# rknightion/iq-to-audio

Hardware: AMD Instinct MI355X
Metric: complex IQ MS/s end-to-end (ingest->48 kHz audio) (higher is better)
Workload: dtype i8; 1 GPU; BASELINE config 2: synthetic 60 s @ 10 MS/s int16 I/Q, 1 NFM channel, +25 kHz, bw 12.5 kHz, D=104, 6401 taps, chunk 4194304; frames_per_gpu=600000000, parallelism=1 independent capture(s), one per GPU; RCCL gather of 48 kHz audio only, audio_samples_48k=2879996, mix_sign=1, settle_steps=55

## Files before the change

### iq-to-audio_amd/csrc/demod_fused.hip

```cpp
#include "common.h"

namespace iqa {

constexpr int SC_THREADS = 256;
constexpr int SC_ITEMS = 8;
constexpr int SC_TILE = SC_THREADS * SC_ITEMS;

struct Aff {
    double A, B;
};
__device__ __forceinline__ Aff then(const Aff &l, const Aff &r) { return Aff{r.A * l.A, fma(r.A, l.B, r.B)}; }

__device__ __forceinline__ Aff wave_inclusive(Aff v, int lane)
{
#pragma unroll
    for (int o = 1; o < kWave; o <<= 1) {
        const double la = __shfl_up(v.A, o, kWave);
        const double lb = __shfl_up(v.B, o, kWave);
        if (lane >= o) v = then(Aff{la, lb}, v);
    }
    return v;
}

__device__ __forceinline__ long long lower_bound_ll(const long long *arr, long long n, long long v)
{
    long long lo = 0, hi = n;
    while (lo < hi) {
        const long long mid = (lo + hi) >> 1;
        if (arr[mid] < v) lo = mid + 1; else hi = mid;
    }
    return lo;
}

enum FOp { F_DEEMPH = 0, F_DC = 1, F_AGC = 2 };
enum FSrc { S_F32 = 0, S_QUAD = 1, S_ENV = 2, S_REAL = 3 };
enum FSink { K_PLAIN = 0, K_CLIP = 1 };

struct FusedArgs {
    const float2 *z;
    const float *x;
    float *y;
    long long n;
    double p0, p1;
    const float2 *prev;
    const double *st;
    const long long *segs;
    long long n_segs;
    unsigned int *peak_bits;
    double *sumsq;
    Aff *agg;
    double *carry;
    double *fin;
    int nblocks;
    int z_aligned, y_aligned;
    int fresh;
};

template <int SRC>
__device__ __forceinline__ float src_value(float2 zc, float2 zp)
{
    if constexpr (SRC == S_QUAD) {
        const float re = zc.x * zp.x + zc.y * zp.y;
        const float im = zc.y * zp.x - zc.x * zp.y;
        return atan2f(im, re);
    } else if constexpr (SRC == S_ENV) {
        return np_abs_c64(zc.x, zc.y);
    } else {
        return zc.x;
    }
}


__global__ void k_quadrature(const float2 *z, long long n, const float2 *prev, float *out)
{
    const long long i = static_cast<long long>(blockIdx.x) * blockDim.x + threadIdx.x;
    if (i >= n) return;
    out[i] = src_value<S_QUAD>(z[i], (i == 0) ? prev[0] : z[i - 1]);
}

__global__ void k_store_last(const float2 *z, long long n, float2 *prev)
{
    if (threadIdx.x == 0 && blockIdx.x == 0) prev[0] = z[n - 1];
}

__global__ void k_envelope(const float2 *z, long long n, float *out)
{
    const long long i = static_cast<long long>(blockIdx.x) * blockDim.x + threadIdx.x;
    if (i < n) out[i] = src_value<S_ENV>(z[i], z[i]);
}

__global__ void k_real(const float2 *z, long long n, float *out)
{
    const long long i = static_cast<long long>(blockIdx.x) * blockDim.x + threadIdx.x;
    if (i < n) out[i] = src_value<S_REAL>(z[i], z[i]);
}


template <int OP, int SRC>
__device__ __forceinline__ void load_u(const FusedArgs &a, long long base, float (&u)[SC_ITEMS], float &u_before)
{
    u_before = 0.f;
    if constexpr (SRC == S_F32) {
#pragma unroll
        for (int i = 0; i < SC_ITEMS; ++i) u[i] = (base + i < a.n) ? a.x[base + i] : 0.f;
        if constexpr (OP == F_DC) {
            if (base == 0) u_before = a.fresh ? 0.f : static_cast<float>(a.st[0]);
            else if (base - 1 < a.n) u_before = a.x[base - 1];
        }
    } else {
        float2 zz[SC_ITEMS + 2];
        static_assert(SC_ITEMS == 8, "the vector path below moves 8 float2 = 4 x 16 bytes per thread");
        const int lane = threadIdx.x & 63;
        const long long wave_base = base - static_cast<long long>(lane) * SC_ITEMS;
        if (a.z_aligned && wave_base + 64 * SC_ITEMS <= a.n) {
            const float4 *p = reinterpret_cast<const float4 *>(a.z + base);
            const float4 q0 = p[0], q1 = p[1], q2 = p[2], q3 = p[3];
            zz[2] = make_float2(q0.x, q0.y);
            zz[3] = make_float2(q0.z, q0.w);
            zz[4] = make_float2(q1.x, q1.y);
            zz[5] = make_float2(q1.z, q1.w);
            zz[6] = make_float2(q2.x, q2.y);
            zz[7] = make_float2(q2.z, q2.w);
            zz[8] = make_float2(q3.x, q3.y);
            zz[9] = make_float2(q3.z, q3.w);
            float2 e0 = make_float2(0.f, 0.f), e1 = make_float2(0.f, 0.f);
            if (lane == 0 && base >= 2) {
                e0 = a.z[base - 2];
                e1 = a.z[base - 1];
            }
            zz[0] = make_float2(__shfl_up(q3.x, 1, kWave), __shfl_up(q3.y, 1, kWave));
            zz[1] = make_float2(__shfl_up(q3.z, 1, kWave), __shfl_up(q3.w, 1, kWave));
            if (lane == 0) {
                zz[0] = e0;
                zz[1] = e1;
            }
        } else {
#pragma unroll
            for (int i = 0; i < SC_ITEMS + 2; ++i) {
                const long long k = base - 2 + i;
                zz[i] = (k >= 0 && k < a.n) ? a.z[k] : make_float2(0.f, 0.f);
            }
        }
        if constexpr (SRC == S_QUAD) {
            if (base == 0) zz[1] = a.fresh ? make_float2(1.f, 0.f) : a.prev[0];
        }
#pragma unroll
        for (int i = 0; i < SC_ITEMS; ++i) u[i] = (base + i < a.n) ? src_value<SRC>(zz[i + 2], zz[i + 1]) : 0.f;
        if constexpr (OP == F_DC) {
            if (base == 0) u_before = a.fresh ? 0.f : static_cast<float>(a.st[0]);
            else u_before = src_value<SRC>(zz[1], zz[0]);
        }
    }
}

template <int OP>
__device__ __forceinline__ Aff fmap(const FusedArgs &a, long long idx, float x, float x_prev, bool maybe_reset)
{
    if constexpr (OP == F_DEEMPH) {
        return Aff{a.p0, a.p1 * static_cast<double>(x)};
    } else if constexpr (OP == F_DC) {
        return Aff{a.p0, static_cast<double>(x - x_prev)};
    } else {
        const float mag = fabsf(x);
        Aff m{1.0, 0.0};
        if (mag > 1e-6f) {
            const float desired = static_cast<float>(a.p0) / mag;
            m = Aff{1.0 - a.p1, a.p1 * static_cast<double>(desired)};
        }
        if (maybe_reset) {
            bool rst = (idx == 0);
            if (!rst && a.segs != nullptr && a.n_segs > 0) {
                const long long lo = lower_bound_ll(a.segs, a.n_segs, idx);
                rst = lo < a.n_segs && a.segs[lo] == idx;
            }
            if (rst) m = Aff{0.0, m.A + m.B};
        }
        return m;
    }
}

__device__ __forceinline__ bool block_has_restart(const FusedArgs &a, long long lo_i, long long hi_i)
{
    if (lo_i == 0) return true;
    if (a.segs == nullptr || a.n_segs <= 0) return false;
    const long long lo = lower_bound_ll(a.segs, a.n_segs, lo_i);
    return lo < a.n_segs && a.segs[lo] < hi_i;
}


template <int THREADS>
__device__ __forceinline__ void sink_count_segments(const FusedArgs &a, long long seg_first, long long first, long long last,
                                                    long long *s_seg)
{
    const int tid = threadIdx.x, lane = tid & 63;
    int c0 = (tid < a.n_segs) && seg_first <= first, c1 = (tid < a.n_segs) && seg_first <= last;
    for (long long kk = tid + THREADS; kk < a.n_segs; kk += THREADS) {
        const long long st = a.segs[kk];
        c0 += st <= first;
        c1 += st <= last;
    }
    c0 = static_cast<int>(wave_sum(static_cast<float>(c0)));
    c1 = static_cast<int>(wave_sum(static_cast<float>(c1)));
    if (lane == 0 && (c0 | c1)) {
        atomicAdd(reinterpret_cast<unsigned long long *>(&s_seg[0]), static_cast<unsigned long long>(c0));
        atomicAdd(reinterpret_cast<unsigned long long *>(&s_seg[1]), static_cast<unsigned long long>(c1));
    }
}

struct SinkPlan {
    bool stats, uniform, simple, general;
    long long seg0, seg1, bnd;
    int sub;
};
__device__ __forceinline__ SinkPlan sink_plan(const FusedArgs &a, bool stats, const long long *s_seg)
{
    SinkPlan p;
    p.stats = stats;
    p.seg0 = stats ? s_seg[0] : -1;
    p.seg1 = stats ? s_seg[1] : -1;
    p.uniform = stats && (p.seg0 == p.seg1);
    p.simple = stats && (p.seg1 == p.seg0 + 1);
    p.general = stats && !p.uniform && !p.simple;
    p.bnd = a.n;
    if (p.simple) p.bnd = a.segs[p.seg1];
    p.sub = blockIdx.x & (IQA_SUMSQ_SLOTS - 1);
    return p;
}

struct SinkAcc {
    float pk = 0.f;
    double run = 0.0, run_hi = 0.0;
    long long seg = 0;
};

template <int SINK>
__device__ __forceinline__ float sink_item(const FusedArgs &a, const SinkPlan &p, SinkAcc &k, float v, long long idx)
{
    if constexpr (SINK != K_CLIP) return v;
    k.pk = fmaxf(k.pk, fabsf(v));
    if (p.stats) {
        const double vv = static_cast<double>(v) * static_cast<double>(v);
        double run = k.run, run_hi = k.run_hi;
        long long seg = k.seg;
        if (p.general) {
            while (seg + 1 < a.n_segs && a.segs[seg + 1] <= idx) {
                if (run != 0.0) atomicAdd(&a.sumsq[seg * IQA_SUMSQ_SLOTS + p.sub], run);
                run = 0.0;
                ++seg;
            }
            run += vv;
        } else {
            const bool low = idx < p.bnd;
            run += low ? vv : 0.0;
            run_hi += low ? 0.0 : vv;
        }
        k.run = run;
        k.run_hi = run_hi;
        k.seg = seg;
    }
    return fminf(fmaxf(v, -0.99f), 0.99f);
}

__device__ __forceinline__ void sink_flush_general(const FusedArgs &a, const SinkPlan &p, SinkAcc &k)
{
    if (p.general && k.run != 0.0) atomicAdd(&a.sumsq[k.seg * IQA_SUMSQ_SLOTS + p.sub], k.run);
    if (p.general) k.run = 0.0;
}

template <int WAVES>
__device__ __forceinline__ void sink_finish(const FusedArgs &a, const SinkPlan &p, SinkAcc &k, float *s_pk, double *s_sq)
{
    const int tid = threadIdx.x, lane = tid & 63, wave = tid >> 6;
    sink_flush_general(a, p, k);
    const float pk = wave_max(k.pk);
    const double wlo = (p.stats && !p.general) ? wave_sum(k.run) : 0.0;
    const double whi = p.simple ? wave_sum(k.run_hi) : 0.0;
    if (lane == 0) {
        s_pk[wave] = pk;
        s_sq[wave] = wlo;
        s_sq[WAVES + wave] = whi;
    }
    __syncthreads();
    if (tid == 0) {
        float m = s_pk[0];
        double lo = s_sq[0], hi = s_sq[WAVES];
#pragma unroll
        for (int w = 1; w < WAVES; ++w) {
            m = fmaxf(m, s_pk[w]);
            lo += s_sq[w];
            hi += s_sq[WAVES + w];
        }
        if (a.peak_bits != nullptr) {
            const unsigned int mb = __float_as_uint(m);
            if (mb > __hip_atomic_load(a.peak_bits, __ATOMIC_RELAXED, __HIP_MEMORY_SCOPE_AGENT)) atomicMax(a.peak_bits, mb);
        }
        if (p.stats && !p.general) atomicAdd(&a.sumsq[p.seg0 * IQA_SUMSQ_SLOTS + p.sub], lo);
        if (p.simple) atomicAdd(&a.sumsq[p.seg1 * IQA_SUMSQ_SLOTS + p.sub], hi);
    }
}

__device__ __forceinline__ void store_items(const FusedArgs &a, long long base, long long lo, long long hi, const float (&vout)[SC_ITEMS])
{
    if (a.y_aligned && base >= lo && base + SC_ITEMS <= hi) {
        float4 *yp = reinterpret_cast<float4 *>(a.y + base);
        yp[0] = make_float4(vout[0], vout[1], vout[2], vout[3]);
        yp[1] = make_float4(vout[4], vout[5], vout[6], vout[7]);
    } else {
#pragma unroll
        for (int i = 0; i < SC_ITEMS; ++i)
            if (base + i >= lo && base + i < hi) a.y[base + i] = vout[i];
    }
}

template <int OP, int SRC>
__global__ __launch_bounds__(SC_THREADS) void k_fused_reduce(FusedArgs a)
{
    __shared__ Aff s_w[SC_THREADS / kWave];
    const int tid = threadIdx.x, lane = tid & 63, wave = tid >> 6;
    const long long blk0 = static_cast<long long>(blockIdx.x) * SC_TILE;
    const long long base = blk0 + static_cast<long long>(tid) * SC_ITEMS;
    const bool mr = (OP == F_AGC) && block_has_restart(a, blk0, blk0 + SC_TILE);
    float u[SC_ITEMS], ub;
    load_u<OP, SRC>(a, base, u, ub);
    Aff t{1.0, 0.0};
#pragma unroll
    for (int i = 0; i < SC_ITEMS; ++i)
        if (base + i < a.n) t = then(t, fmap<OP>(a, base + i, u[i], i ? u[i - 1] : ub, mr));
    const Aff inc = wave_inclusive(t, lane);
    if (lane == kWave - 1) s_w[wave] = inc;
    __syncthreads();
    if (tid == 0) {
        Aff tot = s_w[0];
#pragma unroll
        for (int w = 1; w < SC_THREADS / kWave; ++w) tot = then(tot, s_w[w]);
        a.agg[blockIdx.x] = tot;
    }
}

constexpr int FC_THREADS = 1024;
template <int OP>
__global__ __launch_bounds__(FC_THREADS) void k_fused_carry(FusedArgs a)
{
    __shared__ Aff s_w[FC_THREADS / kWave];
    const int tid = threadIdx.x, lane = tid & 63, wave = tid >> 6;
    double s0;
    if constexpr (OP == F_DEEMPH) s0 = a.fresh ? 0.0 : a.st[0];
    else if constexpr (OP == F_DC) s0 = a.fresh ? 0.0 : a.st[1];
    else s0 = 1.0;
    const int per = (a.nblocks + FC_THREADS - 1) / FC_THREADS;
    const int b0 = tid * per;
    Aff t{1.0, 0.0};
    for (int i = 0; i < per; ++i)
        if (b0 + i < a.nblocks) t = then(t, a.agg[b0 + i]);
    const Aff inc = wave_inclusive(t, lane);
    if (lane == kWave - 1) s_w[wave] = inc;
    __syncthreads();
    Aff pre{1.0, 0.0};
    for (int w = 0; w < wave; ++w) pre = then(pre, s_w[w]);
    Aff exl{__shfl_up(inc.A, 1, kWave), __shfl_up(inc.B, 1, kWave)};
    if (lane == 0) exl = Aff{1.0, 0.0};
    const Aff ex = then(pre, exl);
    double s = fma(ex.A, s0, ex.B);
    for (int i = 0; i < per; ++i) {
        const int b = b0 + i;
        if (b < a.nblocks) {
            a.carry[b] = s;
            const Aff v = a.agg[b];
            s = fma(v.A, s, v.B);
        }
    }
    if (tid == FC_THREADS - 1) a.fin[0] = s;
    if (a.fresh) {
        if (tid == 0 && a.peak_bits != nullptr) a.peak_bits[0] = 0u;
        if (a.sumsq != nullptr)
            for (long long i = tid; i < a.n_segs * IQA_SUMSQ_SLOTS; i += FC_THREADS) a.sumsq[i] = 0.0;
    }
    if (tid == 0) {
        if (a.prev != nullptr) reinterpret_cast<float2 *>(a.fin + 1)[0] = a.fresh ? make_float2(1.f, 0.f) : a.prev[0];
        if (a.st != nullptr) a.fin[2] = a.fresh ? 0.0 : a.st[0];
    }
}

template <int OP, int SRC, int SINK>
__global__ __launch_bounds__(SC_THREADS) void k_fused_apply(FusedArgs a, float2 *prev_out, double *st_out)
{
    __shared__ Aff s_w[SC_THREADS / kWave];
    __shared__ float s_pk[SC_THREADS / kWave];
    __shared__ double s_sq[2 * (SC_THREADS / kWave)];
    __shared__ long long s_seg[2];
    const int tid = threadIdx.x, lane = tid & 63, wave = tid >> 6;
    const long long blk0 = static_cast<long long>(blockIdx.x) * SC_TILE;
    const long long base = blk0 + static_cast<long long>(tid) * SC_ITEMS;
    const bool mr = (OP == F_AGC) && block_has_restart(a, blk0, blk0 + SC_TILE);
    const bool stats = (SINK == K_CLIP) && a.sumsq != nullptr && a.n_segs > 0;
    const double carry_in = a.carry[blockIdx.x];
    long long seg_first = 0;
    if (stats && tid < a.n_segs) seg_first = a.segs[tid];
    if (stats && tid < 2) s_seg[tid] = -1;
    float u[SC_ITEMS], ub;
    load_u<OP, SRC>(a, base, u, ub);
    constexpr bool KEEP = (OP == F_AGC);
    Aff m[KEEP ? SC_ITEMS : 1];
    Aff t{1.0, 0.0};
#pragma unroll
    for (int i = 0; i < SC_ITEMS; ++i) {
        const Aff mi = (base + i < a.n) ? fmap<OP>(a, base + i, u[i], i ? u[i - 1] : ub, mr) : Aff{1.0, 0.0};
        if constexpr (KEEP) m[i] = mi;
        t = then(t, mi);
    }
    if (stats) {
        __syncthreads();
        const long long first = blk0, last = min(blk0 + SC_TILE, a.n) - 1;
        int c0 = (tid < a.n_segs) && seg_first <= first, c1 = (tid < a.n_segs) && seg_first <= last;
        for (long long kk = tid + SC_THREADS; kk < a.n_segs; kk += SC_THREADS) {
            const long long st = a.segs[kk];
            c0 += st <= first;
            c1 += st <= last;
        }
        c0 = static_cast<int>(wave_sum(static_cast<float>(c0)));
        c1 = static_cast<int>(wave_sum(static_cast<float>(c1)));
        if (lane == 0 && (c0 | c1)) {
            atomicAdd(reinterpret_cast<unsigned long long *>(&s_seg[0]), static_cast<unsigned long long>(c0));
            atomicAdd(reinterpret_cast<unsigned long long *>(&s_seg[1]), static_cast<unsigned long long>(c1));
        }
    }
    const Aff inc = wave_inclusive(t, lane);
    if (lane == kWave - 1) s_w[wave] = inc;
    __syncthreads();
    const double ea = __shfl_up(inc.A, 1, kWave), eb = __shfl_up(inc.B, 1, kWave);
    Aff ex = (lane == 0) ? Aff{1.0, 0.0} : Aff{ea, eb};
    Aff wpre{1.0, 0.0};
    for (int w = 0; w < wave; ++w) wpre = then(wpre, s_w[w]);
    ex = then(wpre, ex);
    double s = fma(ex.A, carry_in, ex.B);

    const long long seg0 = stats ? s_seg[0] : -1, seg1 = stats ? s_seg[1] : -1;
    const bool uniform = stats && (seg0 == seg1);
    const bool simple = stats && (seg1 == seg0 + 1);
    const bool general = stats && !uniform && !simple;
    long long bnd = a.n;
    if (simple) bnd = a.segs[seg1];
    long long seg = seg0;
    if (general && base < a.n) seg = lower_bound_ll(a.segs, a.n_segs, base + 1) - 1;
    float pk = 0.f;
    double run = 0.0, run_hi = 0.0;
    float vout[SC_ITEMS];
#pragma unroll
    for (int i = 0; i < SC_ITEMS; ++i) {
        const long long idx = base + i;
        Aff mi;
        if constexpr (KEEP) mi = m[i];
        else mi = (idx < a.n) ? fmap<OP>(a, idx, u[i], i ? u[i - 1] : ub, mr) : Aff{1.0, 0.0};
        s = fma(mi.A, s, mi.B);
        vout[i] = 0.f;
        if (idx < a.n) {
            const float v = (OP == F_AGC) ? u[i] * static_cast<float>(s) : static_cast<float>(s);
            if constexpr (SINK == K_CLIP) {
                pk = fmaxf(pk, fabsf(v));
                vout[i] = fminf(fmaxf(v, -0.99f), 0.99f);
                if (stats) {
                    const double vv = static_cast<double>(v) * static_cast<double>(v);
                    if (general) {
                        while (seg + 1 < a.n_segs && a.segs[seg + 1] <= idx) {
                            if (run != 0.0) atomicAdd(&a.sumsq[seg * IQA_SUMSQ_SLOTS + (blockIdx.x & (IQA_SUMSQ_SLOTS - 1))], run);
                            run = 0.0;
                            ++seg;
                        }
                        run += vv;
                    } else {
                        run += idx < bnd ? vv : 0.0;
                        run_hi += idx < bnd ? 0.0 : vv;
                    }
                }
            } else {
                vout[i] = v;
            }
        }
    }
    if constexpr (SINK == K_CLIP) {
        if (general && run != 0.0) atomicAdd(&a.sumsq[seg * IQA_SUMSQ_SLOTS + (blockIdx.x & (IQA_SUMSQ_SLOTS - 1))], run);
        pk = wave_max(pk);
        const double wlo = (stats && !general) ? wave_sum(run) : 0.0;
        const double whi = simple ? wave_sum(run_hi) : 0.0;
        if (lane == 0) {
            s_pk[wave] = pk;
            s_sq[wave] = wlo;
            s_sq[4 + wave] = whi;
        }
        __syncthreads();
        if (tid == 0) {
            if (a.peak_bits != nullptr) {
                const unsigned int m = __float_as_uint(fmaxf(fmaxf(s_pk[0], s_pk[1]), fmaxf(s_pk[2], s_pk[3])));
                if (m > __hip_atomic_load(a.peak_bits, __ATOMIC_RELAXED, __HIP_MEMORY_SCOPE_AGENT)) atomicMax(a.peak_bits, m);
            }
            const int sub = blockIdx.x & (IQA_SUMSQ_SLOTS - 1);
            if (stats && !general) atomicAdd(&a.sumsq[seg0 * IQA_SUMSQ_SLOTS + sub], s_sq[0] + s_sq[1] + s_sq[2] + s_sq[3]);
            if (simple) atomicAdd(&a.sumsq[seg1 * IQA_SUMSQ_SLOTS + sub], s_sq[4] + s_sq[5] + s_sq[6] + s_sq[7]);
        }
    }
    if (OP != F_AGC && blockIdx.x == a.nblocks - 1 && tid == 0) {
        if constexpr (SRC == S_QUAD) prev_out[0] = a.z[a.n - 1];
        if constexpr (OP == F_DEEMPH) {
            st_out[0] = a.fin[0];
        } else if constexpr (OP == F_DC) {
            float last;
            if constexpr (SRC == S_F32) last = a.x[a.n - 1];
            else last = src_value<SRC>(a.z[a.n - 1], make_float2(0.f, 0.f));
            st_out[0] = static_cast<double>(last);
            st_out[1] = a.fin[0];
        }
    }
    if (a.y_aligned && base + SC_ITEMS <= a.n) {
        float4 *yp = reinterpret_cast<float4 *>(a.y + base);
        yp[0] = make_float4(vout[0], vout[1], vout[2], vout[3]);
        yp[1] = make_float4(vout[4], vout[5], vout[6], vout[7]);
    } else {
#pragma unroll
        for (int i = 0; i < SC_ITEMS; ++i)
            if (base + i < a.n) a.y[base + i] = vout[i];
    }
}

constexpr int FW_THREADS = 256;
constexpr int FW_ROUNDS = 4;
constexpr int FW_WAVES = FW_THREADS / kWave;
constexpr long long FW_ROUND = static_cast<long long>(FW_THREADS) * SC_ITEMS;
constexpr long long FW_SPAN = FW_ROUND * FW_ROUNDS;

static int scan_window(double alpha, long long *window)
{
    if (!(alpha > 0.0 && alpha < 1.0)) return 1;
    const double need = 64.0 * log(2.0) / -log(alpha);
    if (!(need < static_cast<double>(FW_SPAN))) return 1;
    long long w = 512 * static_cast<long long>(ceil(need / 512.0));
    if (w < 512) w = 512;
    while (w > 512 && pow(alpha, static_cast<double>(w - 512)) <= 0x1p-64) w -= 512;
    while (pow(alpha, static_cast<double>(w)) > 0x1p-64) w += 512;
    if (2 * w > FW_SPAN) return 1;
    *window = w;
    return 0;
}

template <int SRC>
__device__ __forceinline__ double windowed_round(const FusedArgs &a, long long base, long long end, bool skip0, Aff *s_w,
                                                 double &s_run, float (&u)[SC_ITEMS])
{
    const int lane = threadIdx.x & 63, wave = threadIdx.x >> 6;
    float ub;
    load_u<F_DEEMPH, SRC>(a, base, u, ub);
    if (skip0 && base == 0) u[0] = 0.f;
    Aff t{1.0, 0.0};
#pragma unroll
    for (int i = 0; i < SC_ITEMS; ++i)
        if (base + i < end) t = then(t, fmap<F_DEEMPH>(a, base + i, u[i], 0.f, false));
    const Aff inc = wave_inclusive(t, lane);
    if (lane == kWave - 1) s_w[wave] = inc;
    __syncthreads();
    const double ea = __shfl_up(inc.A, 1, kWave), eb = __shfl_up(inc.B, 1, kWave);
    Aff ex = (lane == 0) ? Aff{1.0, 0.0} : Aff{ea, eb};
    Aff acc{1.0, 0.0}, wpre{1.0, 0.0};
#pragma unroll
    for (int w = 0; w < FW_WAVES; ++w) {
        if (w == wave) wpre = acc;
        acc = then(acc, s_w[w]);
    }
    ex = then(wpre, ex);
    const double s = fma(ex.A, s_run, ex.B);
    s_run = fma(acc.A, s_run, acc.B);
    return s;
}

__global__ __launch_bounds__(FC_THREADS) void k_fused_clear(float *state, unsigned int *peak_bits, double *sumsq, long long n_sums)
{
    if (state != nullptr && threadIdx.x < 8) state[threadIdx.x] = threadIdx.x ? 0.f : 1.f;
    if (threadIdx.x == 0 && peak_bits != nullptr) peak_bits[0] = 0u;
    if (sumsq != nullptr)
        for (long long i = threadIdx.x; i < n_sums; i += FC_THREADS) sumsq[i] = 0.0;
}

template <int SRC, int SINK>
__global__ __launch_bounds__(FW_THREADS) void k_fused_windowed(FusedArgs a, long long window, float2 *prev_out, double *st_out)
{
    __shared__ Aff s_w[2][FW_WAVES];
    __shared__ float s_pk[FW_WAVES];
    __shared__ double s_sq[2 * FW_WAVES];
    __shared__ long long s_seg[2];
    const int tid = threadIdx.x;
    const long long own = FW_SPAN - window;
    const long long own0 = static_cast<long long>(blockIdx.x) * own, own1 = min(own0 + own, a.n);
    const long long start = blockIdx.x ? own0 - window : 0;
    const bool skip0 = blockIdx.x != 0;
    const bool stats = (SINK == K_CLIP) && a.sumsq != nullptr && a.n_segs > 0;
    double s_run = (blockIdx.x == 0 && !a.fresh) ? a.st[0] : 0.0;
    long long seg_first = 0;
    if (stats && tid < a.n_segs) seg_first = a.segs[tid];
    if (stats && tid < 2) s_seg[tid] = -1;
    if (stats) {
        __syncthreads();
        sink_count_segments<FW_THREADS>(a, seg_first, own0, own1 - 1, s_seg);
    }
    SinkPlan plan{};
    SinkAcc acc;
    for (int r = 0; r < FW_ROUNDS; ++r) {
        const long long rbase = start + r * FW_ROUND;
        if (rbase >= own1) break;
        const long long base = rbase + static_cast<long long>(tid) * SC_ITEMS;
        float u[SC_ITEMS];
        double s = windowed_round<SRC>(a, base, own1, skip0, s_w[r & 1], s_run, u);
        if (r == 0) plan = sink_plan(a, stats, s_seg);
        if (base + SC_ITEMS <= own0 || base >= own1) continue;
        acc.seg = plan.seg0;
        if (plan.general) acc.seg = lower_bound_ll(a.segs, a.n_segs, max(base, own0) + 1) - 1;
        float vout[SC_ITEMS];
#pragma unroll
        for (int i = 0; i < SC_ITEMS; ++i) {
            const long long idx = base + i;
            if (idx < own1) {
                const Aff mi = fmap<F_DEEMPH>(a, idx, u[i], 0.f, false);
                s = fma(mi.A, s, mi.B);
            }
            vout[i] = 0.f;
            if (idx >= own0 && idx < own1) vout[i] = sink_item<SINK>(a, plan, acc, static_cast<float>(s), idx);
        }
        sink_flush_general(a, plan, acc);
        store_items(a, base, own0, own1, vout);
    }
    if constexpr (SINK == K_CLIP) sink_finish<FW_WAVES>(a, plan, acc, s_pk, s_sq);
    if (blockIdx.x != 0) return;
    if (a.nblocks > 1) {
        const long long t0 = (a.n - window) & ~7LL;
        s_run = 0.0;
        __syncthreads();
        for (int r = 0; t0 + r * FW_ROUND < a.n; ++r) {
            float u[SC_ITEMS];
            windowed_round<SRC>(a, t0 + r * FW_ROUND + static_cast<long long>(tid) * SC_ITEMS, a.n, false, s_w[r & 1], s_run, u);
        }
    }
    if (tid == 0) {
        if constexpr (SRC == S_QUAD) prev_out[0] = a.z[a.n - 1];
        st_out[0] = s_run;
    }
}

template <int OP, int SRC, int SINK>
static int launch_fused(FusedArgs a, float2 *prev_out, double *st_out, void *work, hipStream_t s)
{
    if constexpr (OP == F_DEEMPH) {
        long long window;
        if (scan_window(a.p0, &window) == 0) {
            const long long own = FW_SPAN - window;
            a.nblocks = static_cast<int>((a.n + own - 1) / own);
            if (a.fresh && (a.peak_bits != nullptr || a.sumsq != nullptr))
                hipLaunchKernelGGL(k_fused_clear, dim3(1), dim3(FC_THREADS), 0, s, static_cast<float *>(nullptr), a.peak_bits, a.sumsq,
                                   a.n_segs * IQA_SUMSQ_SLOTS);
            hipLaunchKernelGGL((k_fused_windowed<SRC, SINK>), dim3(a.nblocks), dim3(FW_THREADS), 0, s, a, window, prev_out, st_out);
            return check_launch("windowed demodulator");
        }
    }
    a.nblocks = static_cast<int>((a.n + SC_TILE - 1) / SC_TILE);
    char *w = static_cast<char *>(work);
    a.agg = reinterpret_cast<Aff *>(w);
    a.carry = reinterpret_cast<double *>(w + sizeof(Aff) * a.nblocks);
    a.fin = a.carry + a.nblocks;
    hipLaunchKernelGGL((k_fused_reduce<OP, SRC>), dim3(a.nblocks), dim3(SC_THREADS), 0, s, a);
    hipLaunchKernelGGL((k_fused_carry<OP>), dim3(1), dim3(FC_THREADS), 0, s, a);
    FusedArgs b = a;
    b.prev = reinterpret_cast<const float2 *>(a.fin + 1);
    b.st = a.fin + 2;
    b.fresh = 0;
    hipLaunchKernelGGL((k_fused_apply<OP, SRC, SINK>), dim3(a.nblocks), dim3(SC_THREADS), 0, s, b, prev_out, st_out);
    return check_launch("fused demodulator");
}

}

using namespace iqa;

static int demodulate(const iqa_demod_params *p, const void *z_dev, int64_t n, void *state_dev, const void *seg_starts_dev,
                      int64_t n_segs, void *peak_dev, void *sumsq_dev, void *audio_out_dev, void *scratch_dev, void *work_dev,
                      void *stream, int fresh)
{
    if (p == nullptr) return fail_inval("params is NULL");
    if (n < 0 || n_segs < 0) return fail_inval("negative length");
    if (p->mode < IQA_DEMOD_NFM || p->mode > IQA_DEMOD_LSB) return fail_inval("Unsupported demod mode");
    if (n == 0) return IQA_OK;
    if (!z_dev || !state_dev || !audio_out_dev || !work_dev) return fail_inval("NULL device pointer");
    if (n_segs > 0 && !seg_starts_dev) return fail_inval("seg_starts is NULL");
    hipStream_t s = as_stream(stream);
    char *st = static_cast<char *>(state_dev);
    FusedArgs a{};
    a.fresh = fresh;
    a.z = static_cast<const float2 *>(z_dev);
    a.n = n;
    a.segs = static_cast<const long long *>(seg_starts_dev);
    a.n_segs = n_segs;
    a.peak_bits = static_cast<unsigned int *>(peak_dev);
    a.sumsq = static_cast<double *>(sumsq_dev);
    a.y = static_cast<float *>(audio_out_dev);
    a.z_aligned = (reinterpret_cast<uintptr_t>(z_dev) & 15) == 0;
    a.y_aligned = (reinterpret_cast<uintptr_t>(audio_out_dev) & 15) == 0;
    a.prev = reinterpret_cast<const float2 *>(st);
    if (p->mode == IQA_DEMOD_NFM) {
        a.p0 = p->deemph_alpha;
        a.p1 = 1.0 - p->deemph_alpha;
        a.st = reinterpret_cast<const double *>(st + 8);
        return launch_fused<F_DEEMPH, S_QUAD, K_CLIP>(a, reinterpret_cast<float2 *>(st), reinterpret_cast<double *>(st + 8),
                                                      work_dev, s);
    }
    if (!(p->dc_radius > 0.0 && p->dc_radius < 1.0)) return fail_inval("radius must be between 0 and 1");
    a.p0 = static_cast<double>(static_cast<float>(p->dc_radius));
    a.st = reinterpret_cast<const double *>(st + 16);
    double *dc_out = reinterpret_cast<double *>(st + 16);
    if (p->mode == IQA_DEMOD_AM) return launch_fused<F_DC, S_ENV, K_CLIP>(a, nullptr, dc_out, work_dev, s);
    if (!p->agc_enabled) return launch_fused<F_DC, S_REAL, K_CLIP>(a, nullptr, dc_out, work_dev, s);
    if (!scratch_dev) return fail_inval("SSB with AGC needs a float scratch buffer of n elements");
    FusedArgs d = a;
    d.y = static_cast<float *>(scratch_dev);
    d.y_aligned = (reinterpret_cast<uintptr_t>(scratch_dev) & 15) == 0;
    d.peak_bits = nullptr;
    d.sumsq = nullptr;
    int rc = launch_fused<F_DC, S_REAL, K_PLAIN>(d, nullptr, dc_out, work_dev, s);
    if (rc != IQA_OK) return rc;
    FusedArgs g = a;
    g.z = nullptr;
    g.x = static_cast<const float *>(scratch_dev);
    g.p0 = static_cast<double>(static_cast<float>(p->agc_target));
    g.p1 = static_cast<double>(static_cast<float>(p->agc_decay));
    g.st = nullptr;
    return launch_fused<F_AGC, S_F32, K_CLIP>(g, nullptr, nullptr, work_dev, s);
}

extern "C" int iqa_demodulate(const iqa_demod_params *p, const void *z_dev, int64_t n, void *state_dev,
                              const void *seg_starts_dev, int64_t n_segs, void *peak_dev, void *sumsq_dev,
                              void *audio_out_dev, void *scratch_dev, void *work_dev, void *stream)
{
    return demodulate(p, z_dev, n, state_dev, seg_starts_dev, n_segs, peak_dev, sumsq_dev, audio_out_dev, scratch_dev, work_dev, stream, 0);
}

extern "C" int iqa_demodulate_from_reset(const iqa_demod_params *p, const void *z_dev, int64_t n, void *state_dev,
                                         const void *seg_starts_dev, int64_t n_segs, void *peak_dev, void *sumsq_dev,
                                         void *audio_out_dev, void *scratch_dev, void *work_dev, void *stream)
{
    if (n == 0) return fail_inval("iqa_demodulate_from_reset needs samples (an empty block resets nothing)");
    return demodulate(p, z_dev, n, state_dev, seg_starts_dev, n_segs, peak_dev, sumsq_dev, audio_out_dev, scratch_dev, work_dev, stream, 1);
}

extern "C" int iqa_demod_reset(void *state_dev, void *peak_dev, void *sumsq_dev, int64_t n_sums, void *stream)
{
    if (n_sums < 0) return fail_inval("negative length");
    if (!state_dev) return fail_inval("NULL device pointer");
    if (n_sums > 0 && !sumsq_dev) return fail_inval("sumsq is NULL");
    hipLaunchKernelGGL(k_fused_clear, dim3(1), dim3(FC_THREADS), 0, as_stream(stream), static_cast<float *>(state_dev),
                       static_cast<unsigned int *>(peak_dev), static_cast<double *>(sumsq_dev), (long long)n_sums);
    return check_launch("k_fused_clear");
}

extern "C" int iqa_scan_window(double alpha, int64_t *window, int64_t *span)
{
    long long w = 0;
    if (scan_window(alpha, &w) != 0) return 1;
    if (window != nullptr) *window = w;
    if (span != nullptr) *span = FW_SPAN;
    return 0;
}

extern "C" int64_t iqa_scan_workspace_bytes(int64_t n)
{
    const int64_t nb = (n + SC_TILE - 1) / SC_TILE;
    return nb * (sizeof(Aff) + sizeof(double)) + 64;
}


static FusedArgs stage_args(const void *x_dev, int64_t n, void *y_dev)
{
    FusedArgs a{};
    a.x = static_cast<const float *>(x_dev);
    a.y = static_cast<float *>(y_dev);
    a.n = n;
    a.y_aligned = (reinterpret_cast<uintptr_t>(y_dev) & 15) == 0;
    return a;
}

extern "C" int iqa_deemphasis(const void *x_dev, int64_t n, double alpha, void *state_dev, void *y_dev,
                              void *work_dev, void *stream)
{
    if (n < 0) return fail_inval("negative length");
    if (n == 0) return IQA_OK;
    if (!x_dev || !state_dev || !y_dev || !work_dev) return fail_inval("NULL device pointer");
    FusedArgs a = stage_args(x_dev, n, y_dev);
    a.p0 = alpha;
    a.p1 = 1.0 - alpha;
    a.st = static_cast<const double *>(state_dev);
    return launch_fused<F_DEEMPH, S_F32, K_PLAIN>(a, nullptr, static_cast<double *>(state_dev), work_dev, as_stream(stream));
}

extern "C" int iqa_dc_block(const void *x_dev, int64_t n, double radius, void *state_dev, void *y_dev,
                            void *work_dev, void *stream)
{
    if (n < 0) return fail_inval("negative length");
    if (!(radius > 0.0 && radius < 1.0)) return fail_inval("radius must be between 0 and 1");
    if (n == 0) return IQA_OK;
    if (!x_dev || !state_dev || !y_dev || !work_dev) return fail_inval("NULL device pointer");
    FusedArgs a = stage_args(x_dev, n, y_dev);
    a.p0 = static_cast<double>(static_cast<float>(radius));
    a.st = static_cast<const double *>(state_dev);
    return launch_fused<F_DC, S_F32, K_PLAIN>(a, nullptr, static_cast<double *>(state_dev), work_dev, as_stream(stream));
}

extern "C" int iqa_agc(const void *x_dev, int64_t n, double target, double decay, const void *reset_starts_dev,
                       int64_t n_resets, void *y_dev, void *work_dev, void *stream)
{
    if (n < 0 || n_resets < 0) return fail_inval("negative length");
    if (n == 0) return IQA_OK;
    if (!x_dev || !y_dev || !work_dev) return fail_inval("NULL device pointer");
    FusedArgs a = stage_args(x_dev, n, y_dev);
    a.p0 = static_cast<double>(static_cast<float>(target));
    a.p1 = static_cast<double>(static_cast<float>(decay));
    a.segs = static_cast<const long long *>(reset_starts_dev);
    a.n_segs = n_resets;
    return launch_fused<F_AGC, S_F32, K_PLAIN>(a, nullptr, nullptr, work_dev, as_stream(stream));
}


extern "C" int iqa_quadrature(const void *z_dev, int64_t n, void *prev_dev, void *out_dev, void *stream)
{
    if (n < 0) return fail_inval("negative length");
    if (n == 0) return IQA_OK;
    if (!z_dev || !prev_dev || !out_dev) return fail_inval("NULL device pointer");
    hipStream_t s = as_stream(stream);
    hipLaunchKernelGGL(k_quadrature, grid1d(n, 256), dim3(256), 0, s, static_cast<const float2 *>(z_dev), (long long)n,
                       static_cast<const float2 *>(prev_dev), static_cast<float *>(out_dev));
    hipLaunchKernelGGL(k_store_last, dim3(1), dim3(1), 0, s, static_cast<const float2 *>(z_dev), (long long)n,
                       static_cast<float2 *>(prev_dev));
    return check_launch("k_quadrature");
}

extern "C" int iqa_envelope(const void *z_dev, int64_t n, void *out_dev, void *stream)
{
    if (n < 0) return fail_inval("negative length");
    if (n == 0) return IQA_OK;
    if (!z_dev || !out_dev) return fail_inval("NULL device pointer");
    hipLaunchKernelGGL(k_envelope, grid1d(n, 256), dim3(256), 0, as_stream(stream), static_cast<const float2 *>(z_dev),
                       (long long)n, static_cast<float *>(out_dev));
    return check_launch("k_envelope");
}

extern "C" int iqa_real_part(const void *z_dev, int64_t n, void *out_dev, void *stream)
{
    if (n < 0) return fail_inval("negative length");
    if (n == 0) return IQA_OK;
    if (!z_dev || !out_dev) return fail_inval("NULL device pointer");
    hipLaunchKernelGGL(k_real, grid1d(n, 256), dim3(256), 0, as_stream(stream), static_cast<const float2 *>(z_dev),
                       (long long)n, static_cast<float *>(out_dev));
    return check_launch("k_real");
}
```

Measured before the change: 1.040 million MS/s.

## Add lean vectorized fast path to windowed deemphasis scan with wave-uniform indexing

Adds a lean path to the windowed deemphasis/clip kernel for waves lying fully inside the owned range. That path uses 32-bit block-relative offsets, 16-byte vector loads and stores, and a specialised clip/stat loop with no per-item bounds or segment checks. Segment-plan values are made scalar with readfirstlane, and the round loop is kept rolled. The aim is to cut VALU, 64-bit index arithmetic and branching in a hot kernel. This adds code complexity and alignment assumptions. Disabling FP contraction in the quadrature discriminator keeps results matching the slow path.

```diff
diff --git a/iq-to-audio_amd/csrc/demod_fused.hip b/iq-to-audio_amd/csrc/demod_fused.hip
--- a/iq-to-audio_amd/csrc/demod_fused.hip
+++ b/iq-to-audio_amd/csrc/demod_fused.hip
@@ -1,4 +1,6 @@
 #include "common.h"
+
+#include <type_traits>
 
 namespace iqa {
 
@@ -60,6 +62,7 @@
 __device__ __forceinline__ float src_value(float2 zc, float2 zp)
 {
     if constexpr (SRC == S_QUAD) {
+#pragma clang fp contract(off)
         const float re = zc.x * zp.x + zc.y * zp.y;
         const float im = zc.y * zp.x - zc.x * zp.y;
         return atan2f(im, re);
@@ -207,6 +210,12 @@
     }
 }
 
+__device__ __forceinline__ long long uniform_ll(long long v)
+{
+    const int lo = __builtin_amdgcn_readfirstlane(static_cast<int>(v)), hi = __builtin_amdgcn_readfirstlane(static_cast<int>(v >> 32));
+    return (static_cast<long long>(hi) << 32) | static_cast<unsigned int>(lo);
+}
+
 struct SinkPlan {
     bool stats, uniform, simple, general;
     long long seg0, seg1, bnd;
@@ -216,8 +225,8 @@
 {
     SinkPlan p;
     p.stats = stats;
-    p.seg0 = stats ? s_seg[0] : -1;
-    p.seg1 = stats ? s_seg[1] : -1;
+    p.seg0 = stats ? uniform_ll(s_seg[0]) : -1;
+    p.seg1 = stats ? uniform_ll(s_seg[1]) : -1;
     p.uniform = stats && (p.seg0 == p.seg1);
     p.simple = stats && (p.seg1 == p.seg0 + 1);
     p.general = stats && !p.uniform && !p.simple;
@@ -542,10 +551,8 @@
 }
 
 template <int SRC>
-__device__ __forceinline__ double windowed_round(const FusedArgs &a, long long base, long long end, bool skip0, Aff *s_w,
-                                                 double &s_run, float (&u)[SC_ITEMS])
-{
-    const int lane = threadIdx.x & 63, wave = threadIdx.x >> 6;
+__device__ __forceinline__ Aff windowed_front(const FusedArgs &a, long long base, long long end, bool skip0, float (&u)[SC_ITEMS])
+{
     float ub;
     load_u<F_DEEMPH, SRC>(a, base, u, ub);
     if (skip0 && base == 0) u[0] = 0.f;
@@ -553,6 +560,35 @@
 #pragma unroll
     for (int i = 0; i < SC_ITEMS; ++i)
         if (base + i < end) t = then(t, fmap<F_DEEMPH>(a, base + i, u[i], 0.f, false));
+    return t;
+}
+
+template <int SRC>
+__device__ __forceinline__ Aff lean_front(const FusedArgs &a, const void *in, int pos, float (&u)[SC_ITEMS])
+{
+    static_assert(SC_ITEMS == 8, "a thread's eight samples are four (complex) or two (real) 16-byte loads");
+    if constexpr (SRC == S_F32) {
+        const float *x = static_cast<const float *>(in) + pos;
+#pragma unroll
+        for (int i = 0; i < SC_ITEMS; ++i) u[i] = x[i];
+    } else {
+        const float4 *p = reinterpret_cast<const float4 *>(static_cast<const float2 *>(in) + pos);
+        const float4 qm = p[-1], q0 = p[0], q1 = p[1], q2 = p[2], q3 = p[3];
+        const float2 zz[SC_ITEMS + 1] = {make_float2(qm.z, qm.w), make_float2(q0.x, q0.y), make_float2(q0.z, q0.w),
+                                         make_float2(q1.x, q1.y), make_float2(q1.z, q1.w), make_float2(q2.x, q2.y),
+                                         make_float2(q2.z, q2.w), make_float2(q3.x, q3.y), make_float2(q3.z, q3.w)};
+#pragma unroll
+        for (int i = 0; i < SC_ITEMS; ++i) u[i] = src_value<SRC>(zz[i + 1], zz[i]);
+    }
+    Aff t{1.0, 0.0};
+#pragma unroll
+    for (int i = 0; i < SC_ITEMS; ++i) t = then(t, fmap<F_DEEMPH>(a, 0, u[i], 0.f, false));
+    return t;
+}
+
+__device__ __forceinline__ double round_scan(const Aff &t, int wave, Aff *s_w, double &s_run)
+{
+    const int lane = threadIdx.x & 63;
     const Aff inc = wave_inclusive(t, lane);
     if (lane == kWave - 1) s_w[wave] = inc;
     __syncthreads();
@@ -585,12 +621,19 @@
     __shared__ float s_pk[FW_WAVES];
     __shared__ double s_sq[2 * FW_WAVES];
     __shared__ long long s_seg[2];
+    constexpr int WAVE_ROUND = kWave * SC_ITEMS;
     const int tid = threadIdx.x;
+    const int wave = __builtin_amdgcn_readfirstlane(tid >> 6);
     const long long own = FW_SPAN - window;
     const long long own0 = static_cast<long long>(blockIdx.x) * own, own1 = min(own0 + own, a.n);
     const long long start = blockIdx.x ? own0 - window : 0;
     const bool skip0 = blockIdx.x != 0;
     const bool stats = (SINK == K_CLIP) && a.sumsq != nullptr && a.n_segs > 0;
+    const int e_own0 = static_cast<int>(own0 - start), e_own1 = static_cast<int>(own1 - start);
+    int e_bnd = static_cast<int>(FW_SPAN);
+    const bool in_vec = (SRC == S_F32) || a.z_aligned;
+    const void *in = (SRC == S_F32) ? static_cast<const void *>(a.x + start) : static_cast<const void *>(a.z + start);
+    float *out = a.y + start;
     double s_run = (blockIdx.x == 0 && !a.fresh) ? a.st[0] : 0.0;
     long long seg_first = 0;
     if (stats && tid < a.n_segs) seg_first = a.segs[tid];
@@ -601,17 +644,52 @@
     }
     SinkPlan plan{};
     SinkAcc acc;
+#pragma unroll 1
     for (int r = 0; r < FW_ROUNDS; ++r) {
-        const long long rbase = start + r * FW_ROUND;
-        if (rbase >= own1) break;
-        const long long base = rbase + static_cast<long long>(tid) * SC_ITEMS;
+        const int rpos = r * static_cast<int>(FW_ROUND);
+        if (rpos >= e_own1) break;
+        const int wpos = rpos + wave * WAVE_ROUND, pos = rpos + tid * SC_ITEMS;
+        const long long base = start + pos;
+        const bool lean = in_vec && (start != 0 || wpos != 0) && wpos + WAVE_ROUND <= e_own1;
         float u[SC_ITEMS];
-        double s = windowed_round<SRC>(a, base, own1, skip0, s_w[r & 1], s_run, u);
-        if (r == 0) plan = sink_plan(a, stats, s_seg);
+        const Aff t = lean ? lean_front<SRC>(a, in, pos, u) : windowed_front<SRC>(a, base, own1, skip0, u);
+        double s = round_scan(t, wave, s_w[r & 1], s_run);
+        if (r == 0) {
+            plan = sink_plan(a, stats, s_seg);
+            e_bnd = static_cast<int>(min(max(plan.bnd - start, 0LL), FW_SPAN));
+        }
+        if (lean && wpos + WAVE_ROUND <= e_own0) continue;
+        float vout[SC_ITEMS];
+        const bool high = wpos >= e_bnd;
+        if (lean && wpos >= e_own0 && a.y_aligned && !plan.general && (high || wpos + WAVE_ROUND <= e_bnd)) {
+            double side = high ? acc.run_hi : acc.run;
+            auto walk = [&](auto with_stats) {
+#pragma unroll
+                for (int i = 0; i < SC_ITEMS; ++i) {
+                    const Aff mi = fmap<F_DEEMPH>(a, 0, u[i], 0.f, false);
+                    s = fma(mi.A, s, mi.B);
+                    const float v = static_cast<float>(s);
+                    if constexpr (SINK == K_CLIP) {
+                        acc.pk = fmaxf(acc.pk, fabsf(v));
+                        if constexpr (decltype(with_stats)::value) side += static_cast<double>(v) * static_cast<double>(v);
+                        vout[i] = fminf(fmaxf(v, -0.99f), 0.99f);
+                    } else {
+                        vout[i] = v;
+                    }
+                }
+            };
+            if (plan.stats) walk(std::true_type{});
+            else walk(std::false_type{});
+            if (high) acc.run_hi = side;
+            else acc.run = side;
+            float4 *yp = reinterpret_cast<float4 *>(out + pos);
+            yp[0] = make_float4(vout[0], vout[1], vout[2], vout[3]);
+            yp[1] = make_float4(vout[4], vout[5], vout[6], vout[7]);
+            continue;
+        }
         if (base + SC_ITEMS <= own0 || base >= own1) continue;
         acc.seg = plan.seg0;
         if (plan.general) acc.seg = lower_bound_ll(a.segs, a.n_segs, max(base, own0) + 1) - 1;
-        float vout[SC_ITEMS];
 #pragma unroll
         for (int i = 0; i < SC_ITEMS; ++i) {
             const long long idx = base + i;
@@ -633,7 +711,8 @@
         __syncthreads();
         for (int r = 0; t0 + r * FW_ROUND < a.n; ++r) {
             float u[SC_ITEMS];
-            windowed_round<SRC>(a, t0 + r * FW_ROUND + static_cast<long long>(tid) * SC_ITEMS, a.n, false, s_w[r & 1], s_run, u);
+            const Aff t = windowed_front<SRC>(a, t0 + r * FW_ROUND + static_cast<long long>(tid) * SC_ITEMS, a.n, false, u);
+            round_scan(t, wave, s_w[r & 1], s_run);
         }
     }
     if (tid == 0) {
diff --git a/profiles/asm_loop_counts.py b/profiles/asm_loop_counts.py
--- /dev/null
+++ b/profiles/asm_loop_counts.py
@@ -0,0 +1,132 @@
+#!/usr/bin/env python3
+from __future__ import annotations
+
+import re
+import sys
+from collections import Counter
+
+CLASSES = ["valu", "f64", "salu", "branch", "exec", "lane", "cnd", "cmp64", "add64", "mov64", "vmem", "lds", "smem"]
+NOT_SALU = ("s_waitcnt", "s_nop", "s_branch", "s_cbranch", "s_barrier", "s_endpgm", "s_load", "s_buffer_load", "s_sleep",
+            "s_setprio", "s_sendmsg", "s_code_end", "s_setpc", "s_swappc", "s_getpc", "s_inst_prefetch", "s_clause")
+
+
+def classes_of(op: str) -> list[str]:
+    out = []
+    if op.startswith("v_"):
+        out.append("valu")
+        if op.endswith("_f64") or "_f64_" in op:
+            out.append("f64")
+        if op.startswith(("v_readlane", "v_writelane")):
+            out.append("lane")
+        if op.startswith("v_cndmask"):
+            out.append("cnd")
+        if re.match(r"v_cmpx?_\w+_[iu]64", op):
+            out.append("cmp64")
+        if op.startswith("v_lshl_add_u64"):
+            out.append("add64")
+        if op.startswith("v_mov_b64"):
+            out.append("mov64")
+    elif op.startswith(("global_", "buffer_", "flat_", "scratch_")):
+        out.append("vmem")
+    elif op.startswith("ds_"):
+        out.append("lds")
+    elif op.startswith(("s_load", "s_buffer_load")):
+        out.append("smem")
+    elif op.startswith(("s_branch", "s_cbranch")):
+        out.append("branch")
+    elif op.startswith("s_") and not op.startswith(NOT_SALU):
+        out.append("salu")
+        if "saveexec" in op:
+            out.append("exec")
+    return out
+
+
+def fmt(c: Counter) -> str:
+    return "  ".join(f"{k} {c[k]}" for k in CLASSES)
+
+
+def kernels(text: str):
+    lines = text.splitlines()
+    starts = [(i, m.group(1)) for i, l in enumerate(lines) if (m := re.match(r"^(_Z\w+):", l))]
+    for n, (i, name) in enumerate(starts):
+        end = starts[n + 1][0] if n + 1 < len(starts) else len(lines)
+        chunk = lines[i + 1:end]
+        stop = next((k for k, l in enumerate(chunk) if l.strip().startswith(".Lfunc_end")), len(chunk))
+        yield name, chunk[:stop], chunk[stop:]
+
+
+def report(name: str, body: list[str], trailer: list[str], blocks: bool, path: list[str] | None = None) -> None:
+    res = {}
+    for l in trailer:
+        m = re.match(r";\s*(NumVgprs|NumAgprs|NumSgprs|TotalNumSgprs|ScratchSize|Occupancy|LDSByteSize):\s*(\d+)", l.strip())
+        if m:
+            res.setdefault(m.group(1), m.group(2))
+    ins = []
+    label_at = {}
+    for l in body:
+        t = l.split(";")[0].strip()
+        if not t or t.startswith("."):
+            m = re.match(r"^(\.LBB\w+):", t)
+            if m:
+                label_at[m.group(1)] = len(ins)
+            continue
+        m = re.match(r"^(\.LBB\w+):", t)
+        if m:
+            label_at[m.group(1)] = len(ins)
+            continue
+        parts = t.split()
+        op = parts[0]
+        tgt = parts[1] if op.startswith(("s_branch", "s_cbranch")) and len(parts) > 1 else None
+        ins.append((op, tgt))
+    print(f"== {name}")
+    print("   " + "  ".join(f"{k} {v}" for k, v in res.items()))
+
+    def count(lo: int, hi: int) -> Counter:
+        c = Counter()
+        for op, _ in ins[lo:hi]:
+            c.update(classes_of(op))
+        return c
+
+    print(f"   whole kernel ({len(ins)} instructions): {fmt(count(0, len(ins)))}")
+    if path:
+        ends = sorted(set(label_at.values()) | {len(ins)})
+        total = Counter()
+        for lab in path:
+            lo = label_at[lab if lab.startswith(".") else ".LBB" + lab]
+            total.update(count(lo, next(e for e in ends if e > lo)))
+        print(f"   path {' '.join(path)} (sum of these blocks, each up to the next label): {fmt(total)}")
+    loops = {}
+    for i, (op, tgt) in enumerate(ins):
+        if tgt in label_at and label_at[tgt] <= i:
+            lo = label_at[tgt]
+            loops[tgt] = (lo, max(i + 1, loops.get(tgt, (0, 0))[1]))
+    order = sorted(loops.items(), key=lambda kv: kv[1][0])
+    for lab, (lo, hi) in order:
+        outer = not any(o != lab and olo <= lo and hi <= ohi for o, (olo, ohi) in loops.items())
+        bar = sum(1 for op, _ in ins[lo:hi] if op == "s_barrier")
+        print(f"   loop {lab}{'' if outer else ' (nested)'}: {hi - lo} instructions, {bar} barriers: {fmt(count(lo, hi))}")
+        if blocks and outer:
+            cuts = sorted({lo, hi} | {v for v in label_at.values() if lo < v < hi})
+            names = {v: k for k, v in label_at.items()}
+            for b0, b1 in zip(cuts, cuts[1:]):
+                c = count(b0, b1)
+                to = [t for _, t in ins[b0:b1] if t]
+                print(f"      {names.get(b0, '(entry)'):>14} {b1 - b0:5d}: valu {c['valu']:4d} f64 {c['f64']:3d} salu {c['salu']:3d} "
+                      f"vmem {c['vmem']:2d} lds {c['lds']:2d} lane {c['lane']:2d} -> {' '.join(to)}")
+
+
+def main() -> int:
+    args = [a for a in sys.argv[1:] if not a.startswith("--")]
+    path = next((a.split("=", 1)[1].split(",") for a in sys.argv[1:] if a.startswith("--path=")), None)
+    if len(args) != 2:
+        print(__doc__)
+        return 2
+    text = open(args[0]).read()
+    for name, body, trailer in kernels(text):
+        if args[1] in name:
+            report(name, body, trailer, "--blocks" in sys.argv, path)
+    return 0
+
+
+if __name__ == "__main__":
+    sys.exit(main())
```

After: 1.058 million MS/s (median of 3 runs). No clear change (+1.7%).
